# shubhamchandak94/HARC

Hardware: AMD Instinct MI355X
Metric: Mreads/s reorder+encode, 100 bp (higher is better)
Workload: dtype u64 (2-bit packed bases, XOR+popcount)

## Files before the change

### harc_amd/csrc/internal.h

```cpp
#pragma once
#include <hip/hip_runtime.h>
#include <stdint.h>
#include <stdio.h>
#include <string.h>
#include <map>
#include <string>
#include <utility>
#include <vector>
#include "../../include/harc_amd.h"

#define HARC_NONE 0xFFFFFFFFu
#define HARC_MAXW 8
#define HARC_MAXW3 12
#define HARC_MAXK (1u << 20)
#define HARC_LOOK_CHUNKS 16
#ifndef HARC_NSUGG
#define HARC_NSUGG 8
#endif

void harc_set_error(const char *fmt, ...);

#define HIP_TRY(expr)                                                                                          \
    do {                                                                                                       \
        hipError_t _e = (expr);                                                                                \
// ... 126 lines not shown
void harc_pool_release(harc_amd_ctx *c, harc_mark_t m);
struct PoolScope {
    harc_amd_ctx *c; harc_mark_t mk; bool armed = true;
    explicit PoolScope(harc_amd_ctx *c_) : c(c_), mk(harc_pool_mark(c_)) {}
    PoolScope(const PoolScope &) = delete;
    PoolScope &operator=(const PoolScope &) = delete;
    ~PoolScope() { if (armed) harc_pool_release(c, mk); }
    void keep() { armed = false; }
    void release_now() { if (armed) { harc_pool_release(c, mk); armed = false; } }
};

int prim_sort_pairs_u64_u32(harc_amd_ctx *c, const uint64_t *kin, uint64_t *kout, const uint32_t *vin, uint32_t *vout, size_t n, unsigned end_bit);
#define BL_TILE_WORDS 16384u
#define BL_PART_BITS 20
#define harc_bitmap_tiles(nwords) ((uint32_t)(((uint64_t)(nwords) + BL_TILE_WORDS - 1) / BL_TILE_WORDS))
#define harc_bitmap_item(w, b0, b1) (((uint64_t)((((uint32_t)(w) % BL_TILE_WORDS) << 10) | ((uint32_t)(b0) << 5) | (uint32_t)(b1)) << BL_PART_BITS) | (uint64_t)((uint32_t)(w) / BL_TILE_WORDS))
int harc_bitmap_from_items(harc_amd_ctx *c, const uint64_t *items, uint64_t *tmp, size_t n, uint64_t nwords, uint32_t *bitmap);
int prim_sort_keys_u64(harc_amd_ctx *c, const uint64_t *kin, uint64_t *kout, size_t n, unsigned end_bit);
int prim_excl_scan_u32(harc_amd_ctx *c, const uint32_t *in, uint32_t *out, size_t n);
int prim_excl_scan_u32_to_u64(harc_amd_ctx *c, const uint32_t *in, uint64_t *out, size_t n);
int prim_excl_scan_u8_to_u64(harc_amd_ctx *c, const uint8_t *in, uint64_t *out, size_t n);
int prim_incl_scan_u64(harc_amd_ctx *c, const uint64_t *in, uint64_t *out, size_t n);
int prim_incl_max_u32(harc_amd_ctx *c, const uint32_t *in, uint32_t *out, size_t n);
int prim_incl_max_u64(harc_amd_ctx *c, const uint64_t *in, uint64_t *out, size_t n);

int s1_pack_ascii(harc_amd_ctx *c, const char *d_ascii, uint32_t n, uint32_t stride, uint64_t *d_out);
int s1_pack3_ascii(harc_amd_ctx *c, const char *d_ascii, uint32_t n, uint32_t stride, uint64_t *d_out);
int s1_unpack_to_ascii(harc_amd_ctx *c, const uint64_t *d_reads, uint32_t n, char *d_out);
int s1_bucket_reads(harc_amd_ctx *c, const uint64_t *d_packed, uint32_t n, uint32_t nb, uint32_t *d_out);
int s1_partition_reads(harc_amd_ctx *c, const uint64_t *d_packed, uint32_t n, uint32_t nb, uint64_t *d_out, unsigned long long *d_counts);
int shard_partition(harc_amd_ctx *c, const uint64_t *d_words, uint32_t n, int nwords, bool three_bit, uint32_t nb, uint32_t gid0,
                    uint64_t *d_out, uint32_t *d_gid_out, unsigned long long *d_counts);
int shard_map_ids(harc_amd_ctx *c, uint32_t *d_v, uint64_t n, const uint32_t *d_map, uint32_t nmap, unsigned int *d_err);
int stage1_run(harc_amd_ctx *c);
int stage1_make_oriented(harc_amd_ctx *c, uint32_t i0 = 0, uint32_t i1 = 0xFFFFFFFFu);
int s1_orient(harc_amd_ctx *c, const uint64_t *reads, const uint32_t *order, const uint8_t *rc, uint32_t m, uint64_t *out);
int harc_dict_alloc(harc_amd_ctx *c, DictDev *d, uint32_t n, uint64_t cap_like);
int harc_dict_build(harc_amd_ctx *c, DictDev *d, uint64_t *keys, uint32_t *ids, uint32_t n, unsigned kbits);
void harc_dict_free(harc_amd_ctx *c, DictDev *d);
int stage2_run(harc_amd_ctx *c);
int pack_order_run(harc_amd_ctx *c);

static inline std::vector<uint8_t> &out_buf(harc_amd_ctx *c, int id, int shard) { harc_amd_ctx::OutBuf &o = c->out[std::make_pair(id, shard)]; o.ptr = nullptr; o.len = 0; return o.own; }
static inline void out_slice(harc_amd_ctx *c, int id, int shard, const void *p, size_t n) { harc_amd_ctx::OutBuf &o = c->out[std::make_pair(id, shard)]; o.own.clear(); o.ptr = (const uint8_t *)p; o.len = n; }
int harc_host_alloc(harc_amd_ctx *c, void **p, size_t bytes);
void harc_host_reset(harc_amd_ctx *c);
int harc_d2h(harc_amd_ctx *c, std::vector<uint8_t> &dst, const void *d_src, size_t bytes);

int build_line_index(harc_amd_ctx *c, const char *d_txt, uint64_t nbytes, const uint64_t **nls_out, uint64_t *total_lines_out);

int write_shard_family(harc_amd_ctx *c, const std::string &od, int first_shard, int e_lo = 0, int e_hi = -1);
int write_whole_job_files(harc_amd_ctx *c, const std::string &od);

struct BgzfCand { uint64_t off; uint32_t bsize, hdr, isize, crc; };
struct BgzfMember { uint64_t cdata, text; uint32_t clen, isize, crc, hdr; };
struct BgzfPlan { std::vector<BgzfMember> m; uint64_t text = 0, next = 0; };
int harc_bgzf_plan(harc_amd_ctx *c, const uint8_t *d_in, uint64_t n, uint64_t start, uint64_t own_end, uint64_t base_off, BgzfPlan *plan);
int harc_bgzf_run(harc_amd_ctx *c, const uint8_t *d_in, const BgzfPlan &plan, uint64_t base_off, char *d_out);

struct BgzfOutStats { uint64_t text = 0, bytes = 0, members = 0, stored = 0; double seconds = 0; };
int harc_bgzf_deflate(harc_amd_ctx *c, const char *d_text, uint64_t n_bytes, int32_t flags, uint8_t *d_out, uint64_t out_capacity, uint64_t *n_out, BgzfOutStats *st);
// ... 1 lines not shown
```

### harc_amd/csrc/prims.hip

```cpp
#include "devutil.h"
#include <rocprim/rocprim.hpp>

int harc_tmp_reserve(harc_amd_ctx *c, size_t bytes)
{
    if (bytes <= c->tmp_bytes) return HARC_AMD_OK;
    if (c->d_tmp) harc_raw_free(c, c->d_tmp);
    c->d_tmp = nullptr; c->tmp_bytes = 0;
    size_t want = bytes + (bytes >> 3) + 4096;
    RC_TRY(harc_raw_alloc(c, &c->d_tmp, want));
    c->tmp_bytes = want;
    return HARC_AMD_OK;
}

#define PRIM_CALL(call_with_tmp)                                \
    do {                                                        \
        size_t bytes = 0; void *tmp = nullptr;                  \
        HIP_TRY(call_with_tmp);                                 \
        RC_TRY(harc_tmp_reserve(c, bytes));                     \
        tmp = c->d_tmp; bytes = c->tmp_bytes;                   \
        HIP_TRY(call_with_tmp);                                 \
    } while (0)

int prim_sort_pairs_u64_u32(harc_amd_ctx *c, const uint64_t *kin, uint64_t *kout, const uint32_t *vin, uint32_t *vout, size_t n, unsigned end_bit)
{
// ... 32 lines not shown

int prim_excl_scan_u8_to_u64(harc_amd_ctx *c, const uint8_t *in, uint64_t *out, size_t n)
{
    if (n == 0) return HARC_AMD_OK;
    auto it = rocprim::make_transform_iterator(in, u8_to_u64());
    PRIM_CALL(rocprim::exclusive_scan(tmp, bytes, it, out, (uint64_t)0, n, rocprim::plus<uint64_t>(), c->stream));
    return HARC_AMD_OK;
}

int prim_incl_scan_u64(harc_amd_ctx *c, const uint64_t *in, uint64_t *out, size_t n)
{
    if (n == 0) return HARC_AMD_OK;
    PRIM_CALL(rocprim::inclusive_scan(tmp, bytes, in, out, n, rocprim::plus<uint64_t>(), c->stream));
    return HARC_AMD_OK;
}

int prim_incl_max_u32(harc_amd_ctx *c, const uint32_t *in, uint32_t *out, size_t n)
{
    if (n == 0) return HARC_AMD_OK;
    PRIM_CALL(rocprim::inclusive_scan(tmp, bytes, in, out, n, rocprim::maximum<uint32_t>(), c->stream));
    return HARC_AMD_OK;
}

int prim_incl_max_u64(harc_amd_ctx *c, const uint64_t *in, uint64_t *out, size_t n)
{
    if (n == 0) return HARC_AMD_OK;
    PRIM_CALL(rocprim::inclusive_scan(tmp, bytes, in, out, n, rocprim::maximum<uint64_t>(), c->stream));
    return HARC_AMD_OK;
}

__global__ void k_selftest_grid(uint64_t n, unsigned long long *out)
{
    const uint64_t i = harc_gid();
    unsigned long long one = i < n ? 1ULL : 0ULL, idx = i < n ? (unsigned long long)i : 0ULL;
    for (int o = 32; o > 0; o >>= 1) { one += __shfl_xor(one, o, 64); idx += __shfl_xor(idx, o, 64); }
    if ((threadIdx.x & 63) == 0 && one) { atomicAdd(&out[0], one); atomicAdd(&out[1], idx); }
}
__global__ void k_selftest_grid32(uint32_t n, unsigned long long *out)
{
    const uint32_t i = harc_gid32();
    unsigned long long one = i < n ? 1ULL : 0ULL, idx = i < n ? (unsigned long long)i : 0ULL;
    for (int o = 32; o > 0; o >>= 1) { one += __shfl_xor(one, o, 64); idx += __shfl_xor(idx, o, 64); }
    if ((threadIdx.x & 63) == 0 && one) { atomicAdd(&out[0], one); atomicAdd(&out[1], idx); }
}
__global__ void k_selftest_fold(uint64_t n, unsigned long long *out)
{
    const uint64_t wave = harc_bid() * 4 + (threadIdx.x >> 6);
    const int lane = threadIdx.x & 63;
    const uint64_t i = wave * 16 + (uint64_t)(lane >> 2);
    const bool mine = i < n && (lane & 3) == 0;
// ... 27 lines not shown
```

### harc_amd/csrc/stage1.hip

```cpp
#include "devutil.h"
#include <stdlib.h>
#include <type_traits>

struct S1Args {
    int L, maxmatch, thresh, maxsearch, Lp;
    int ds[2], de[2], kbits[2];
    uint32_t N, K;
    const uint64_t *reads;
    HashSlot *slots[2];
    uint64_t cap[2];
    const uint32_t *ids[2];
    int firstmax;
    const uint32_t *bloom[2]; uint32_t bloom_lines; int bloom_nwin[2]; uint32_t bloom_mmask;
    const uint2 *largetab;
    uint64_t *mirror;
    unsigned long long *claimed;
    uint32_t *bid;
    ChainHdr *hdr;
    uint4 *cnt;
    uint2 *steps;
    uint8_t *need;
    uint32_t *seedbuf;
    uint32_t *needrank;
    uint32_t *rmeta;
// ... 166 lines not shown
{
    const uint64_t gid = harc_gid();
    if (gid >= (uint64_t)n * W) return;
    const uint32_t i = (uint32_t)(gid / W); const int w = (int)(gid % W);
    out[gid] = reads[(size_t)idx[i] * W + w];
}
int s1_partition_reads(harc_amd_ctx *c, const uint64_t *d_packed, uint32_t n, uint32_t nb, uint64_t *d_out, unsigned long long *d_counts)
{
    HIP_TRY(hipMemsetAsync(d_counts, 0, (size_t)nb * 8, c->stream));
    if (!n) { HIP_TRY(hipStreamSynchronize(c->stream)); return HARC_AMD_OK; }
    PoolScope scope(c);
    uint32_t *b = nullptr, *i0 = nullptr, *i1 = nullptr; uint64_t *k0 = nullptr, *k1 = nullptr;
    RC_TRY(dalloc(c, &b, n)); RC_TRY(dalloc(c, &i0, n)); RC_TRY(dalloc(c, &i1, n)); RC_TRY(dalloc(c, &k0, n)); RC_TRY(dalloc(c, &k1, n));
    hipLaunchKernelGGL(k_bucket, harc_grid256(n), dim3(256), 0, c->stream, d_packed, n, c->P.readlen, c->W, nb, b);
    hipLaunchKernelGGL(k_bucket_keys, harc_grid256(n), dim3(256), 0, c->stream, (const uint32_t *)b, n, k0, i0, d_counts);
    unsigned bits = 1; while ((1u << bits) < nb) bits++;
    RC_TRY(prim_sort_pairs_u64_u32(c, k0, k1, i0, i1, n, bits));
    hipLaunchKernelGGL(k_gather_reads, harc_grid256((uint64_t)n * c->W), dim3(256), 0, c->stream, d_packed, (const uint32_t *)i1, n, c->W, d_out);
    HIP_TRY(hipGetLastError());
    HIP_TRY(hipStreamSynchronize(c->stream));
    return HARC_AMD_OK;
}

template <int W> __global__ void k_keygen2(const uint64_t *reads, uint32_t n, int off0, int nbits0, int off1, int nbits1, uint64_t *keys0, uint64_t *keys1, uint32_t *ids)
{
    const uint32_t i = harc_gid32();
    if (i >= n) return;
    uint64_t r[W];
#pragma unroll
    for (int w = 0; w < W; w++) r[w] = reads[(size_t)i * W + w];
    {
        const int wi = off0 >> 6, sh = off0 & 63;
        const uint64_t lo = sel0<W>(r, wi), hi = sel0<W>(r, wi + 1);
        uint64_t v = sh ? ((lo >> sh) | (hi << (64 - sh))) : lo;
        if (nbits0 < 64) v &= ((uint64_t)1 << nbits0) - 1;
        keys0[i] = v;
    }
    {
        const int wi = off1 >> 6, sh = off1 & 63;
        const uint64_t lo = sel0<W>(r, wi), hi = sel0<W>(r, wi + 1);
        uint64_t v = sh ? ((lo >> sh) | (hi << (64 - sh))) : lo;
        if (nbits1 < 64) v &= ((uint64_t)1 << nbits1) - 1;
        keys1[i] = v;
    }
    ids[i] = i;
}
__global__ void k_large_sizes(const unsigned long long *list, uint32_t nlist, HashSlot *s0, HashSlot *s1, uint32_t *sz)
{
    const uint32_t b = harc_gid32();
    if (b >= nlist) return;
    const unsigned long long e = list[b];
    const HashSlot *slot = ((e & 1) ? s1 : s0) + (e >> 1);
    sz[b] = slot->count & SLOT_CNT_MASK;
}
template <int W> __global__ __launch_bounds__(64) void k_large_fill(const unsigned long long *list, uint32_t nlist, HashSlot *s0, HashSlot *s1, const uint32_t *ids0, const uint32_t *ids1,
                                                                   const uint64_t *moff, const uint64_t *reads, uint2 *largetab, uint64_t *mirror)
{
    const uint32_t b = blockIdx.y * gridDim.x + blockIdx.x;
    if (b >= nlist) return;
    const int lane = threadIdx.x;
    const unsigned long long e = list[b];
    const int l = (int)(e & 1);
    HashSlot *slot = (l ? s1 : s0) + (e >> 1);
    const uint32_t st = slot->start, cnt = slot->count & SLOT_CNT_MASK;
    const uint32_t *ids = (l ? ids1 : ids0) + st;
    const uint64_t m0 = moff[b];
    for (uint32_t k = lane; k < cnt; k += 64) {
        const uint32_t rid = ids[k];
#pragma unroll
        for (int w = 0; w < W; w++) mirror[(m0 + k) * W + w] = reads[(size_t)rid * W + w];
    }
    if (lane == 0) { largetab[b] = make_uint2(st, (uint32_t)m0); slot->start = b; }
}
__global__ void k_mark_heads(const uint64_t *skeys, uint32_t n, uint32_t *head)
{
    const uint32_t i = harc_gid32();
    if (i >= n) return;
    head[i] = (i == 0 || skeys[i] != skeys[i - 1]) ? 1u : 0u;
}
__global__ void k_bin_starts(const uint32_t *head, const uint32_t *binidx, uint32_t n, uint32_t *binstart, uint32_t *nbins, const uint64_t *skeys, uint64_t cap, uint64_t *v)
{
    const uint32_t i = harc_gid32();
    if (i >= n) return;
    if (head[i]) { const uint32_t b = binidx[i]; binstart[b] = i; v[b] = bucket_slot(skeys[i], cap) + (uint64_t)n - (uint64_t)b; }
    if (i == n - 1) *nbins = binidx[i] + head[i];
}
#define HARC_LARGEBIN 16u
#define HARC_STEP_CAP 12
#define HARC_BO_FREE 1u
#define HARC_BO_CAP 3u
#define HARC_SCAN_BUDGET 12
#define MIXED_MAX (1u << 20)
#define MIXED_BUDGET 200000u
__device__ __forceinline__ uint64_t rotl64(uint64_t x, unsigned r) { r &= 63u; return r ? (x << r) | (x >> (64u - r)) : x; }
__global__ void k_mixed_find(const uint64_t *rk, uint32_t n, unsigned sbits, uint64_t *sk, uint32_t *list, unsigned int *meta)
{
    const uint32_t i = harc_gid32();
    if (i >= n) return;
    const int shift = (int)(64u - sbits);
    const uint64_t b = rotl64(rk[i], 64u - sbits);
    sk[i] = b;
    if (i == 0) return;
    const uint64_t a = rotl64(rk[i - 1], 64u - sbits);
    if (a != b && (a >> shift) == (b >> shift)) { const unsigned int at = atomicAdd(&meta[0], 1u); if (at < MIXED_MAX) list[at] = i; else meta[1] = 1u; }
}
__global__ void k_mixed_own(const uint64_t *sk, int shift, uint32_t *list, unsigned int *meta)
{
    const uint32_t t = harc_gid32();
    const unsigned int nl = meta[0] < MIXED_MAX ? meta[0] : MIXED_MAX;
    if (t >= nl || meta[1]) return;
    const uint32_t i = list[t];
    const uint64_t top = sk[i] >> shift;
    for (uint32_t h = i; h > 0 && (sk[h - 1] >> shift) == top;) {
        h--;
        if (h > 0 && sk[h] != sk[h - 1] && (sk[h - 1] >> shift) == top) { list[t] = HARC_NONE; return; }
        if (i - h > MIXED_BUDGET) { meta[1] = 1u; return; }
    }
// ... 85 lines not shown
                for (;;) {
                    unsigned long long *mp = reinterpret_cast<unsigned long long *>(&slots[sl]) + 1;
                    if (atomicCAS(mp, 0ULL, meta) == 0ULL) break;
                    if ((sl & 3) == 3) atomicOr(&slots[sl - 3].count, SLOT_OVF);
                    if (++sl == cap) sl = 0;
                }
                slots[sl].key = key;
            } else {
                uint4 w; w.x = (uint32_t)key; w.y = (uint32_t)(key >> 32); w.z = (uint32_t)meta; w.w = (uint32_t)(meta >> 32) | ovf;
                if (tiled) tile[sl - lo] = w; else *reinterpret_cast<uint4 *>(&slots[sl]) = w;
            }
            if (large_list && cnt > HARC_LARGEBIN) {
                const unsigned int at = atomicAdd(large_n, 1u);
                if (at < large_max) large_list[at] = ((unsigned long long)sl << 1) | large_tag;
            }
        }
    }
    if (tiled) {
        __syncthreads();
        for (uint32_t j = threadIdx.x; j < (uint32_t)(hi - lo); j += blockDim.x) *reinterpret_cast<uint4 *>(&slots[lo + j]) = tile[j];
    }
}

__global__ void k_s1_bloom_keys(const uint64_t *keys, uint32_t n, uint32_t nlines, int nwin, uint32_t mmask, uint64_t *pk)
{
    const uint32_t i = harc_gid32();
    if (i >= n) return;
    uint32_t w, m;
    bloom_pos(keys[i], key_scramble(keys[i]), nlines, nwin, mmask, &w, &m);
    const uint32_t b0 = (uint32_t)__ffs((int)m) - 1u, b1 = 31u - (uint32_t)__clz((int)m);
    pk[i] = harc_bitmap_item(w, b0, b1);
}
__global__ __launch_bounds__(256) void k_s1_bloom_tile(const uint64_t *pk, uint32_t n, uint64_t nwords, uint32_t *bloom)
{
    __shared__ uint32_t tile[BL_TILE_WORDS];
    __shared__ uint32_t bounds[2];
    const uint32_t part = blockIdx.x;
    for (uint32_t j = threadIdx.x; j < BL_TILE_WORDS; j += 256) tile[j] = 0u;
    if (threadIdx.x < 2) {
        const uint64_t want = (uint64_t)part + threadIdx.x, pmask = ((uint64_t)1 << BL_PART_BITS) - 1;
        uint32_t lo = 0, hi = n;
        while (lo < hi) { const uint32_t mid = lo + (hi - lo) / 2; if ((pk[mid] & pmask) < want) lo = mid + 1; else hi = mid; }
        bounds[threadIdx.x] = lo;
    }
    __syncthreads();
    for (uint32_t i = bounds[0] + threadIdx.x; i < bounds[1]; i += 256) {
        const uint32_t v = (uint32_t)(pk[i] >> BL_PART_BITS);
        atomicOr(&tile[v >> 10], (1u << ((v >> 5) & 31u)) | (1u << (v & 31u)));
    }
    __syncthreads();
    const uint64_t base = (uint64_t)part * BL_TILE_WORDS;
    for (uint32_t j = threadIdx.x; j < BL_TILE_WORDS; j += 256) if (base + j < nwords) bloom[base + j] = tile[j];
}
int harc_bitmap_from_items(harc_amd_ctx *c, const uint64_t *items, uint64_t *tmp, size_t n, uint64_t nwords, uint32_t *bitmap)
{
// ... 1936 lines not shown
    for (int k = 0; k < W; k++) r[k] = shfl_u64(mine, rl * W + k);
    if (!on) return;
    uint64_t ow = mine;
    if (rev) { rc_words<W>(r, L, o); ow = sel0<W>(o, w); }
    out[(size_t)i * W + w] = ow;
}

int harc_dict_alloc(harc_amd_ctx *c, DictDev *d, uint32_t n, uint64_t cap_like)
{
    d->cap = 0; d->slots = nullptr; d->ids = nullptr; d->d_nbins = nullptr;
    if (n == 0) return HARC_AMD_OK;
    if (cap_like) d->cap = cap_like;
    else {
        unsigned long long m = 4;
        size_t fr = 0, tot = 0;
        if (hipMemGetInfo(&fr, &tot) == hipSuccess) { fr += c->pool_total; while (m > 2 && ((double)m * n * sizeof(HashSlot) > 0.2 * (double)fr || (double)m * n * sizeof(HashSlot) > 0.15 * (double)tot)) m--; }
        if (c->P.table_slots_per_read >= 2 && c->P.table_slots_per_read <= 4) m = (unsigned long long)c->P.table_slots_per_read;
        if (const char *e = getenv("HARC_AMD_CAPMULT")) m = strtoull(e, nullptr, 10);
        d->cap = (((m < 2 ? 2 : m) * n + 4) + 3) & ~3ull;
    }
    RC_TRY(dalloc(c, &d->slots, d->cap)); RC_TRY(dalloc(c, &d->ids, n)); RC_TRY(dalloc(c, &d->d_nbins, 2));
    return HARC_AMD_OK;
}
int harc_dict_build(harc_amd_ctx *c, DictDev *d, uint64_t *keys, uint32_t *ids, uint32_t n, unsigned kbits)
{
    (void)kbits;
    if (n == 0) return HARC_AMD_OK;
    PoolScope scope(c);
    uint64_t *k1 = nullptr; uint32_t *h0 = nullptr, *b0 = nullptr, *bs = nullptr;
    RC_TRY(dalloc(c, &k1, n)); RC_TRY(dalloc(c, &h0, n)); RC_TRY(dalloc(c, &b0, n)); RC_TRY(dalloc(c, &bs, n));
    unsigned sbits = 64;
    { unsigned lg = 1; while (((uint64_t)1 << lg) < n) lg++; sbits = ((lg + 8 + 7) / 8) * 8; if (sbits > 64) sbits = 64; }
    if (const char *e = getenv("HARC_AMD_SORT_BITS")) { const int x = atoi(e); if (x >= 1 && x <= 64) sbits = (unsigned)x; }
    uint32_t *mixed = nullptr; unsigned int *mmeta = nullptr; uint64_t *k2 = nullptr;
    RC_TRY(dalloc(c, &mixed, MIXED_MAX)); RC_TRY(dalloc(c, &mmeta, 4));
    RC_TRY(dalloc(c, &k2, n));
    uint64_t *const k2v = k2;
    hipLaunchKernelGGL(k_scramble_keys, harc_grid256(n), dim3(256), 0, c->stream, keys, n, sbits < 64 ? sbits : 0u);
    uint32_t nbins = 0;
    for (;;) {
        HIP_TRY(hipMemsetAsync(mmeta, 0, 16, c->stream));
        HIP_TRY(hipMemsetAsync(d->d_nbins, 0, 8, c->stream));
        if (sbits < 64) {
            RC_TRY(prim_sort_pairs_u64_u32(c, keys, k2, ids, d->ids, n, sbits));
            hipLaunchKernelGGL(k_mixed_find, harc_grid256(n), dim3(256), 0, c->stream, (const uint64_t *)k2, n, sbits, k1, mixed, mmeta);
            hipLaunchKernelGGL(k_mixed_own, dim3(MIXED_MAX / 256), dim3(256), 0, c->stream, (const uint64_t *)k1, (int)(64 - sbits), mixed, mmeta);
            hipLaunchKernelGGL(k_mixed_fix, dim3(MIXED_MAX / 256), dim3(256), 0, c->stream, k1, d->ids, n, (int)(64 - sbits), (const uint32_t *)mixed, mmeta);
        } else RC_TRY(prim_sort_pairs_u64_u32(c, keys, k1, ids, d->ids, n, 64));
        hipLaunchKernelGGL(k_mark_heads, harc_grid256(n), dim3(256), 0, c->stream, k1, n, h0);
        RC_TRY(prim_excl_scan_u32(c, h0, b0, n));
        hipLaunchKernelGGL(k_bin_starts, harc_grid256(n), dim3(256), 0, c->stream, h0, b0, n, bs, d->d_nbins, (const uint64_t *)k1, d->cap, k2v);
        unsigned int mm[2] = { 0, 0 };
        HIP_TRY(hipMemcpyAsync(&nbins, d->d_nbins, 4, hipMemcpyDeviceToHost, c->stream));
        HIP_TRY(hipMemcpyAsync(mm, mmeta, 8, hipMemcpyDeviceToHost, c->stream));
        HIP_TRY(hipStreamSynchronize(c->stream));
        if (getenv("HARC_AMD_TRACE")) fprintf(stderr, "[index] sort on the top %u bits: %u places where different keys share them%s\n", sbits, mm[0], mm[1] ? " -- too many or too long, sorting on all bits" : "");
        if (!mm[1] || sbits == 64) break;
        hipLaunchKernelGGL(k_rotate_keys, harc_grid256(n), dim3(256), 0, c->stream, keys, n, 64u - sbits);
        sbits = 64;
    }
    const int fill = getenv("HARC_AMD_TABLE_FILL") ? atoi(getenv("HARC_AMD_TABLE_FILL")) != 0 : (uint64_t)nbins * 16 >= d->cap;
    if (!fill) HIP_TRY(hipMemsetAsync(d->slots, 0, d->cap * sizeof(HashSlot), c->stream));
    d->nbins = nbins;
    {
        uint64_t *v = k2v, *q = keys;
        const unsigned gb = (nbins + 255) / 256;
        RC_TRY(prim_incl_max_u64(c, v, q, nbins));
        for (int pass = 0; pass < 2; pass++)
            hipLaunchKernelGGL(k_table_place, dim3(gb), dim3(256), 0, c->stream, (const uint64_t *)k1, (const uint32_t *)d->ids, (const uint32_t *)bs, nbins, n, (const uint64_t *)q,
                               d->slots, d->cap, d->bigthresh, d->large_list, d->large_n, d->large_max, d->large_tag, d->d_nbins, pass, pass == 0 ? 0u : (gb > 64 ? gb - 64 : 0u), fill);
    }
    HIP_TRY(hipGetLastError());
    uint32_t nb2[2] = { 0, 0 };
    HIP_TRY(hipMemcpyAsync(nb2, d->d_nbins, 8, hipMemcpyDeviceToHost, c->stream));
    HIP_TRY(hipStreamSynchronize(c->stream));
    scope.release_now();
    if (nb2[1]) { harc_set_error("dictionary: %u bins hold more than %u reads with the same k-mer (count field of the slot), or lie more than 16384 bins beyond the end of the table", nb2[1], SLOT_CNT_MASK); return HARC_AMD_EINVAL; }
    return HARC_AMD_OK;
}
void harc_dict_free(harc_amd_ctx *c, DictDev *d)
{
    if (d->slots) harc_dev_free(c, d->slots);
    if (d->ids) harc_dev_free(c, d->ids);
    if (d->d_nbins) harc_dev_free(c, d->d_nbins);
    d->slots = nullptr; d->ids = nullptr; d->d_nbins = nullptr; d->cap = 0;
}

__global__ void k_selftest_ids(uint32_t *ids, uint32_t n)
{
    const uint32_t i = harc_gid32();
    if (i < n) ids[i] = i;
}
static int selftest_index(harc_amd_ctx *c, const uint64_t *keys, uint32_t n, uint32_t bigthresh, bool want_large, uint64_t *cap, uint32_t *nbins, void *slots,
                          uint32_t *ids, uint64_t *large, uint64_t large_capacity, uint64_t *n_large)
{
    PoolScope scope(c);
    DictDev d;
    RC_TRY(harc_dict_alloc(c, &d, n, 0));
    const uint64_t room = *cap;
    *cap = d.cap;
    if (!slots) return HARC_AMD_OK;
    if (room < d.cap) { harc_set_error("harc_amd_selftest_index: the table has %llu slots, the caller's buffer %llu", (unsigned long long)d.cap, (unsigned long long)room); return HARC_AMD_EINVAL; }
    uint64_t *k0 = nullptr; uint32_t *i0 = nullptr; unsigned long long *d_large = nullptr; unsigned int *d_nlarge = nullptr;
    const uint32_t maxlarge = 2 * (n / HARC_LARGEBIN) + 16;
    RC_TRY(dalloc(c, &k0, n)); RC_TRY(dalloc(c, &i0, n));
    if (want_large) {
        RC_TRY(dalloc(c, &d_large, maxlarge)); RC_TRY(dalloc(c, &d_nlarge, 4));
        HIP_TRY(hipMemsetAsync(d_nlarge, 0, 16, c->stream));
        d.large_list = d_large; d.large_n = d_nlarge; d.large_max = maxlarge; d.large_tag = 1u;
    }
    d.bigthresh = bigthresh;
    HIP_TRY(hipMemcpyAsync(k0, keys, (size_t)n * 8, hipMemcpyHostToDevice, c->stream));
    hipLaunchKernelGGL(k_selftest_ids, harc_grid256(n), dim3(256), 0, c->stream, i0, n);
    HIP_TRY(hipMemsetAsync(d.slots, 0xA5, d.cap * sizeof(HashSlot), c->stream));
    HIP_TRY(hipMemsetAsync(d.ids, 0xA5, (size_t)n * 4, c->stream));
    RC_TRY(harc_dict_build(c, &d, k0, i0, n, 64));
    *nbins = d.nbins;
    HIP_TRY(hipMemcpyAsync(slots, d.slots, d.cap * sizeof(HashSlot), hipMemcpyDeviceToHost, c->stream));
    HIP_TRY(hipMemcpyAsync(ids, d.ids, (size_t)n * 4, hipMemcpyDeviceToHost, c->stream));
    unsigned int nl = 0;
    if (want_large) HIP_TRY(hipMemcpyAsync(&nl, d_nlarge, 4, hipMemcpyDeviceToHost, c->stream));
    HIP_TRY(hipStreamSynchronize(c->stream));
    if (want_large) {
        *n_large = nl;
        uint64_t take = nl < maxlarge ? nl : maxlarge;
        if (take > large_capacity) take = large_capacity;
        if (take) HIP_TRY(hipMemcpy(large, d_large, (size_t)take * 8, hipMemcpyDeviceToHost));
    }
    return HARC_AMD_OK;
}
extern "C" int harc_amd_selftest_index(harc_amd_ctx *c, const uint64_t *keys, uint64_t n, int32_t slots_per_read, uint32_t bigthresh, int32_t want_large,
                                       uint64_t *cap, uint32_t *nbins, void *slots, uint32_t *ids, uint64_t *large, uint64_t large_capacity, uint64_t *n_large)
{
    if (!c || !cap || n == 0 || n > 0xFFFFFFF0ull || (slots_per_read != 0 && (slots_per_read < 2 || slots_per_read > 4))) { harc_set_error("harc_amd_selftest_index: bad arguments"); return HARC_AMD_EINVAL; }
    if (slots && (!keys || !nbins || !ids || (want_large && (!n_large || (!large && large_capacity))))) { harc_set_error("harc_amd_selftest_index: a NULL output"); return HARC_AMD_EINVAL; }
    HIP_TRY(hipSetDevice(c->P.device));
    const int32_t spr = c->P.table_slots_per_read;
    c->P.table_slots_per_read = slots_per_read;
    const int rc = selftest_index(c, keys, (uint32_t)n, bigthresh, want_large != 0, cap, nbins, slots, ids, large, large_capacity, n_large);
// ... 99 lines not shown
    unsigned long long *d_large = nullptr; unsigned int *d_nlarge = nullptr;
    const uint32_t maxlarge = 2 * (N / HARC_LARGEBIN) + 16;
    if (N) {
        RC_TRY(harc_dict_alloc(c, &dict[0], N, 0)); RC_TRY(harc_dict_alloc(c, &dict[1], N, dict[0].cap));
        ilap("tables allocated");
        RC_TRY(dalloc(c, &d_large, maxlarge)); RC_TRY(dalloc(c, &d_nlarge, 4));
        HIP_TRY(hipMemsetAsync(d_nlarge, 0, 16, c->stream));
        for (int l = 0; l < 2; l++) { dict[l].large_list = d_large; dict[l].large_n = d_nlarge; dict[l].large_max = maxlarge; dict[l].large_tag = (uint32_t)l; }
        dict[0].bigthresh = dict[1].bigthresh = HARC_LARGEBIN;
        if (bloom_bits) {
            uint64_t nl = ((uint64_t)N * (uint64_t)bloom_bits + 511) / 512 + 1;
            if (nl > 0x0FFFFFFFull) nl = 0x0FFFFFFFull;
            bloom_lines = (uint32_t)nl;
            bloom_tiled = getenv("HARC_AMD_S1BLOOM_TILED") ? atoi(getenv("HARC_AMD_S1BLOOM_TILED")) != 0 : (size_t)bloom_lines * 64 >= ((size_t)64 << 20);
            if (((uint64_t)bloom_lines * 16 + BL_TILE_WORDS - 1) / BL_TILE_WORDS + 1 >= ((uint64_t)1 << BL_PART_BITS)) bloom_tiled = false;
            for (int l = 0; l < 2; l++) {
                RC_TRY(dalloc(c, &d_bloom[l], (size_t)bloom_lines * 16)); if (!bloom_tiled) HIP_TRY(hipMemsetAsync(d_bloom[l], 0, (size_t)bloom_lines * 64, c->stream));
                const int nb = P.dict_end[l] - P.dict_start[l] + 1;
                const bool same = P.dict_end[0] - P.dict_start[0] == P.dict_end[1] - P.dict_start[1];
                bloom_nwin[l] = (same && bloom_m > 0 && nb > bloom_m && (size_t)bloom_lines * 64 >= bloom_mz_bytes) ? nb - bloom_m + 1 : 0;
            }
        }
        PoolScope kscope(c);
        uint64_t *kboth[2] = { nullptr, nullptr }; uint32_t *i0 = nullptr;
        RC_TRY(dalloc(c, &kboth[0], N)); RC_TRY(dalloc(c, &kboth[1], N)); RC_TRY(dalloc(c, &i0, N));
        hipLaunchKernelGGL((k_keygen2<W>), harc_grid256(N), dim3(256), 0, c->stream, c->d_reads, N, 2 * P.dict_start[0], 2 * (P.dict_end[0] - P.dict_start[0] + 1),
                           2 * P.dict_start[1], 2 * (P.dict_end[1] - P.dict_start[1] + 1), kboth[0], kboth[1], i0);
        ilap("bitmaps allocated, keys made");
        for (int l = 0; l < 2; l++) {
            const int kbits = 2 * (P.dict_end[l] - P.dict_start[l] + 1);
            uint64_t *const k0 = kboth[l];
            if (bloom_lines && bloom_tiled) {
                PoolScope bscope(c);
                uint64_t *pa = nullptr, *pb = nullptr; RC_TRY(dalloc(c, &pa, (size_t)N + 1)); RC_TRY(dalloc(c, &pb, (size_t)N + 1));
                const uint64_t nwords = (uint64_t)bloom_lines * 16;
                hipLaunchKernelGGL(k_s1_bloom_keys, harc_grid256(N), dim3(256), 0, c->stream, (const uint64_t *)k0, N, bloom_lines, bloom_nwin[l], bloom_mmask, pa);
                RC_TRY(harc_bitmap_from_items(c, pa, pb, N, nwords, d_bloom[l]));
                if (getenv("HARC_AMD_S1BLOOM_VERIFY")) {
                    uint32_t *ref = nullptr; unsigned long long *nd = nullptr, hnd = 0;
                    RC_TRY(dalloc(c, &ref, (size_t)nwords)); RC_TRY(dalloc(c, &nd, 1));
                    HIP_TRY(hipMemsetAsync(ref, 0, (size_t)nwords * 4, c->stream)); HIP_TRY(hipMemsetAsync(nd, 0, 8, c->stream));
                    hipLaunchKernelGGL(k_s1_bloom_set, harc_grid256(N), dim3(256), 0, c->stream, (const uint64_t *)k0, N, ref, bloom_lines, bloom_nwin[l], bloom_mmask);
                    hipLaunchKernelGGL(k_s1_bloom_diff, harc_grid256(nwords), dim3(256), 0, c->stream, (const uint32_t *)ref, (const uint32_t *)d_bloom[l], nwords, nd);
                    HIP_TRY(hipMemcpyAsync(&hnd, nd, 8, hipMemcpyDeviceToHost, c->stream));
                    HIP_TRY(hipStreamSynchronize(c->stream));
                    if (hnd) { harc_set_error("stage I bitmap built by tiles differs from the one built with atomics in %llu words", hnd); return HARC_AMD_EINTERNAL; }
                }
            } else if (bloom_lines) hipLaunchKernelGGL(k_s1_bloom_set, harc_grid256(N), dim3(256), 0, c->stream, (const uint64_t *)k0, N, d_bloom[l], bloom_lines, bloom_nwin[l], bloom_mmask);
            ilap("bitmap built");
            RC_TRY(harc_dict_build(c, &dict[l], k0, i0, N, (unsigned)kbits));
            ilap("table built");
        }
    }
    if (N && P.num_chains <= 0 && P.reads_per_chain <= 0 && (double)dict[0].nbins > 0.98 * (double)N) {
        const uint32_t k2 = N / 256 < 4096 ? N / 256 : 4096;
        if (k2 > K) { K = k2; c->C.chains = K; if (!getenv("HARC_AMD_QUAD")) quad = K <= 16384; }
    }
    uint32_t nlarge = 0;
    if (N) {
        HIP_TRY(hipMemcpyAsync(&nlarge, d_nlarge, 4, hipMemcpyDeviceToHost, c->stream));
        HIP_TRY(hipStreamSynchronize(c->stream));
        if (nlarge > maxlarge) { harc_set_error("stage I: %u bins above %u reads, list of %u", nlarge, HARC_LARGEBIN, maxlarge); return HARC_AMD_EINTERNAL; }
    }
    uint2 *d_largetab = nullptr; uint64_t *d_mirror = nullptr;
    uint32_t *d_sz0 = nullptr, *d_huge = nullptr; unsigned int *d_nhuge = nullptr; uint32_t nhuge = 0;
    uint64_t large_entries = 0;
    if (nlarge) {
        uint32_t *sz = nullptr; uint64_t *moff = nullptr;
        RC_TRY(dalloc(c, &d_largetab, nlarge)); RC_TRY(dalloc(c, &sz, (size_t)nlarge + 1)); RC_TRY(dalloc(c, &moff, (size_t)nlarge + 1));
        HIP_TRY(hipMemsetAsync(sz + nlarge, 0, 4, c->stream));
        hipLaunchKernelGGL(k_large_sizes, harc_grid256(nlarge), dim3(256), 0, c->stream, (const unsigned long long *)d_large, nlarge, dict[0].slots, dict[1].slots, sz);
        d_sz0 = sz;
        RC_TRY(dalloc(c, &d_huge, (size_t)nlarge + 1)); RC_TRY(dalloc(c, &d_nhuge, 4));
// ... 367 lines not shown
```

### harc_amd/csrc/stage2.hip

```cpp
#include "devutil.h"
#include <time.h>
#include <algorithm>
#include <stdlib.h>

#define TUPLE_NONE 0xFFFFFFFFFFFFFFFFULL

struct S2Args {
    int L, W, W3, thresh_s, maxsearch;
    int ds[2], de[2], kbits[2];
    uint32_t M, S, T, q, nC;
    uint64_t total;
    const uint64_t *oreads;
    const uint8_t *flag, *pos, *rc;
    const uint32_t *order;
    const uint64_t *cand3;
    const uint32_t *cand_order;
    uint8_t *head;
    uint64_t *gstart;
    uint8_t *cons;
    const uint32_t *chead;
    const HashSlot *slots[2]; uint64_t cap[2]; const uint32_t *ids[2];
    unsigned long long *best;
    unsigned long long *bestbin[2];
    const uint32_t *bloom[2]; int bloom_shift[2];
// ... 1477 lines not shown
            RC_TRY(dalloc(c, &bloom[0], ((size_t)1 << (lb - 3)) + 1));
            bloom4_tiled = getenv("HARC_AMD_S2BLOOM_TILED") ? atoi(getenv("HARC_AMD_S2BLOOM_TILED")) != 0 : (((size_t)1 << (lb - 3)) * 4 >= ((size_t)64 << 20));
            if ((uint64_t)T * 4 > 0xFFFFFFFFull || harc_bitmap_tiles((uint64_t)1 << (lb - 3)) + 1 >= (1u << BL_PART_BITS)) bloom4_tiled = false;
            if (!bloom4_tiled) HIP_TRY(hipMemsetAsync(bloom[0], 0, ((size_t)1 << (lb - 3)) * 4, c->stream));
            bloom[1] = bloom[0]; bloom_shift[0] = bloom_shift[1] = 64 - lb;
            a.bloom_lbits = lb - 7;
            a.bloom_nwin = (a.kbits[0] / 3 == 21 && !getenv("HARC_AMD_BLOOM4_HASHED")) ? 21 - BLOOM4_M + 1 : 0;
        } else for (int l = 0; l < 2; l++) {
            RC_TRY(dalloc(c, &bloom[l], ((size_t)1 << (lb - 5)) + 1));
            HIP_TRY(hipMemsetAsync(bloom[l], 0, ((size_t)1 << (lb - 5)) * 4, c->stream));
            bloom_shift[l] = 64 - lb;
        }
        PoolScope kscope(c);
        uint64_t *k0 = nullptr; uint32_t *i0k = nullptr; uint64_t *items = nullptr, *items_tmp = nullptr;
        RC_TRY(dalloc(c, &k0, T)); RC_TRY(dalloc(c, &i0k, T));
        const uint64_t b4words = (uint64_t)1 << (lb - 3);
        if (bloom4 && bloom4_tiled) { RC_TRY(dalloc(c, &items, (size_t)T * 4 + 1)); RC_TRY(dalloc(c, &items_tmp, (size_t)T * 4 + 1)); }
        for (int l = 0; l < 2; l++) {
            hipLaunchKernelGGL(k_key3, G256(T), cand3, T, W3, 3 * a.ds[l], a.kbits[l], k0, i0k);
            if (bloom4 && bloom4_tiled) hipLaunchKernelGGL(k_bloom4_items, G256(T), (const uint64_t *)k0, T, a.bloom_lbits, a.bloom_nwin, l, a.kbits[l] / 3, harc_bitmap_tiles(b4words), items + (size_t)l * 2 * T);
            else if (bloom4) hipLaunchKernelGGL(k_bloom4_set, G256(T), (const uint64_t *)k0, T, bloom[0], a.bloom_lbits, a.bloom_nwin, l, a.kbits[l] / 3);
            else hipLaunchKernelGGL(k_bloom_set, G256(T), (const uint64_t *)k0, T, bloom[l], bloom_shift[l]);
            lap("  keys, bitmap items");
            RC_TRY(harc_dict_build(c, &dict[l], k0, i0k, T, (unsigned)a.kbits[l]));
            hipLaunchKernelGGL(k_count_big_bins, G256(dict[l].cap), dict[l].slots, dict[l].cap, (uint32_t)P.maxsearch, d_big);
            lap("  dictionary built");
        }
        if (bloom4 && bloom4_tiled) {
            RC_TRY(harc_bitmap_from_items(c, items, items_tmp, (size_t)T * 4, b4words, bloom[0]));
            lap("  combined bitmap from sorted items");
            if (getenv("HARC_AMD_S2BLOOM_VERIFY")) {
                uint32_t *ref = nullptr; unsigned long long *nd = nullptr, hnd = 0;
                RC_TRY(dalloc(c, &ref, (size_t)b4words + 1)); RC_TRY(dalloc(c, &nd, 1));
                HIP_TRY(hipMemsetAsync(ref, 0, (size_t)b4words * 4, c->stream)); HIP_TRY(hipMemsetAsync(nd, 0, 8, c->stream));
                for (int l = 0; l < 2; l++) {
                    hipLaunchKernelGGL(k_key3, G256(T), cand3, T, W3, 3 * a.ds[l], a.kbits[l], k0, i0k);
                    hipLaunchKernelGGL(k_bloom4_set, G256(T), (const uint64_t *)k0, T, ref, a.bloom_lbits, a.bloom_nwin, l, a.kbits[l] / 3);
                }
                hipLaunchKernelGGL(k_words_differ, harc_grid256(b4words), dim3(256), 0, c->stream, (const uint32_t *)ref, (const uint32_t *)bloom[0], b4words, nd);
                HIP_TRY(hipMemcpyAsync(&hnd, nd, 8, hipMemcpyDeviceToHost, c->stream));
                HIP_TRY(hipStreamSynchronize(c->stream));
                if (hnd) { harc_set_error("stage II bitmap built by tiles differs from the one built with atomics in %llu words", hnd); return HARC_AMD_EINTERNAL; }
            }
        }
        HIP_TRY(hipStreamSynchronize(c->stream));
    }
    for (int l = 0; l < 2; l++) { a.slots[l] = dict[l].slots; a.cap[l] = dict[l].cap; a.ids[l] = dict[l].ids; a.bloom[l] = bloom[l]; a.bloom_shift[l] = bloom_shift[l]; }
// ... 437 lines not shown
```

Before: 695.7.

## Fuse key scrambling and bloom items into keygen, single-pass bin scan in dict build

Stage I key generation now produces the scrambled, rotated sortable keys and the bloom bitmap items (or atomic bloom bits) in the same kernel, so the separate scramble and bloom-key kernels and their extra passes over the key arrays go away. Dictionary building swaps the head-mark, exclusive-scan, bin-start and inclusive-max chain for a custom two-pass wavefront scan that finds bin heads, ranks and the running max of slot offsets together. This cuts kernel launches and global memory traffic, but the bin scan adds a decoupled segment scan that leans on the MIXED scratch buffer and wave-level shuffles, which brings correctness and capacity risks.

```diff
diff --git a/harc_amd/csrc/internal.h b/harc_amd/csrc/internal.h
--- a/harc_amd/csrc/internal.h
+++ b/harc_amd/csrc/internal.h
@@ -172,7 +172,7 @@
 int prim_excl_scan_u8_to_u64(harc_amd_ctx *c, const uint8_t *in, uint64_t *out, size_t n);
 int prim_incl_scan_u64(harc_amd_ctx *c, const uint64_t *in, uint64_t *out, size_t n);
 int prim_incl_max_u32(harc_amd_ctx *c, const uint32_t *in, uint32_t *out, size_t n);
-int prim_incl_max_u64(harc_amd_ctx *c, const uint64_t *in, uint64_t *out, size_t n);
+int prim_bins_scan(harc_amd_ctx *c, const uint64_t *skeys, size_t n, uint64_t cap, uint32_t *binstart, uint64_t *q, uint32_t *nbins, void *scratch, size_t scratch_bytes);
 
 int s1_pack_ascii(harc_amd_ctx *c, const char *d_ascii, uint32_t n, uint32_t stride, uint64_t *d_out);
 int s1_pack3_ascii(harc_amd_ctx *c, const char *d_ascii, uint32_t n, uint32_t stride, uint64_t *d_out);
@@ -186,7 +186,9 @@
 int stage1_make_oriented(harc_amd_ctx *c, uint32_t i0 = 0, uint32_t i1 = 0xFFFFFFFFu);
 int s1_orient(harc_amd_ctx *c, const uint64_t *reads, const uint32_t *order, const uint8_t *rc, uint32_t m, uint64_t *out);
 int harc_dict_alloc(harc_amd_ctx *c, DictDev *d, uint32_t n, uint64_t cap_like);
-int harc_dict_build(harc_amd_ctx *c, DictDev *d, uint64_t *keys, uint32_t *ids, uint32_t n, unsigned kbits);
+enum { HARC_KEYS_RAW = 0, HARC_KEYS_SORTABLE = 1 };
+unsigned harc_dict_sort_bits(uint32_t n);
+int harc_dict_build(harc_amd_ctx *c, DictDev *d, uint64_t *keys, uint32_t *ids, uint32_t n, unsigned kbits, int keys_are);
 void harc_dict_free(harc_amd_ctx *c, DictDev *d);
 int stage2_run(harc_amd_ctx *c);
 int pack_order_run(harc_amd_ctx *c);
diff --git a/harc_amd/csrc/prims.hip b/harc_amd/csrc/prims.hip
--- a/harc_amd/csrc/prims.hip
+++ b/harc_amd/csrc/prims.hip
@@ -78,10 +78,72 @@
     return HARC_AMD_OK;
 }
 
-int prim_incl_max_u64(harc_amd_ctx *c, const uint64_t *in, uint64_t *out, size_t n)
+struct BinPart { long long m; uint32_t c, pad; };
+struct BinPartOp {
+    __host__ __device__ BinPart operator()(const BinPart &a, const BinPart &b) const
+    {
+        const long long bm = b.m - (long long)a.c;
+        return BinPart{ a.m > bm ? a.m : bm, a.c + b.c, 0u };
+    }
+};
+#define BINS_NONE (-(1ll << 62))
+#define BINS_SEG_MIN 2048u
+#define BINS_UNROLL 4
+template <bool WRITE> __global__ __launch_bounds__(256) void k_bins_pass(const uint64_t *k, uint32_t n, uint64_t cap, uint32_t seg, uint32_t nseg, BinPart *part,
+                                                                       uint32_t *binstart, uint64_t *q, uint32_t *nbins)
+{
+    const uint32_t w = (blockIdx.x * 256u + threadIdx.x) >> 6;
+    if (w >= nseg) return;
+    const int lane = threadIdx.x & 63;
+    const unsigned long long below = ((unsigned long long)1 << lane) - 1;
+    uint32_t C = 0; long long M = BINS_NONE;
+    if (WRITE) { C = part[w].c; M = part[w].m; }
+    const uint64_t base = (uint64_t)w * seg, end = base + seg < n ? base + seg : (uint64_t)n;
+    uint64_t carry = base ? k[base - 1] : 0;
+    for (uint64_t at = base; at < end; at += 64u * BINS_UNROLL) {
+        uint64_t key[BINS_UNROLL];
+#pragma unroll
+        for (int u = 0; u < BINS_UNROLL; u++) { const uint64_t i = at + 64u * u + lane; key[u] = i < end ? k[i] : 0; }
+#pragma unroll
+        for (int u = 0; u < BINS_UNROLL; u++) {
+            const uint64_t i = at + 64u * u + lane;
+            uint64_t prev = __shfl_up(key[u], 1, 64);
+            if (lane == 0) prev = carry;
+            carry = __shfl(key[u], 63, 64);
+            const bool head = i < end && (i == 0 || key[u] != prev);
+            const unsigned long long hb = __ballot(head);
+            const uint32_t rank = C + (uint32_t)__popcll(hb & below);
+            long long v = head ? (long long)bucket_slot(key[u], cap) - (long long)rank : BINS_NONE;
+            if (WRITE) {
+                for (int d = 1; d < 64; d <<= 1) { const long long o = __shfl_up(v, d, 64); if (lane >= d && o > v) v = o; }
+                if (M > v) v = M;
+                if (head) { binstart[rank] = (uint32_t)i; q[rank] = (uint64_t)(v + (long long)n); }
+                if (i < end && i + 1 == n) *nbins = rank + (head ? 1u : 0u);
+                M = __shfl(v, 63, 64);
+            } else if (v > M) M = v;
+            C += (uint32_t)__popcll(hb);
+        }
+    }
+    if (!WRITE) {
+        for (int o = 32; o > 0; o >>= 1) { const long long x = __shfl_xor(M, o, 64); if (x > M) M = x; }
+        if (lane == 0) part[w] = BinPart{ M, C, 0u };
+    }
+}
+int prim_bins_scan(harc_amd_ctx *c, const uint64_t *skeys, size_t n, uint64_t cap, uint32_t *binstart, uint64_t *q, uint32_t *nbins, void *scratch, size_t scratch_bytes)
 {
     if (n == 0) return HARC_AMD_OK;
-    PRIM_CALL(rocprim::inclusive_scan(tmp, bytes, in, out, n, rocprim::maximum<uint64_t>(), c->stream));
+    const size_t room = scratch_bytes / (2 * sizeof(BinPart));
+    if (room == 0 || n > 0xFFFFFFFFull || (n + room - 1) / room > (1u << 30) || room > 0x7FFFFFFFull) { harc_set_error("prim_bins_scan: %zu keys, scratch of %zu bytes", n, scratch_bytes); return HARC_AMD_EINVAL; }
+    size_t seg = (n + room - 1) / room;
+    if (seg < BINS_SEG_MIN) seg = BINS_SEG_MIN;
+    seg = (seg + 64 * BINS_UNROLL - 1) / (64 * BINS_UNROLL) * (64 * BINS_UNROLL);
+    const uint32_t nseg = (uint32_t)((n + seg - 1) / seg);
+    BinPart *part = (BinPart *)scratch, *front = part + nseg;
+    const dim3 grid((nseg + 3) / 4);
+    hipLaunchKernelGGL(k_bins_pass<false>, grid, dim3(256), 0, c->stream, skeys, (uint32_t)n, cap, (uint32_t)seg, nseg, part, (uint32_t *)nullptr, (uint64_t *)nullptr, (uint32_t *)nullptr);
+    PRIM_CALL(rocprim::exclusive_scan(tmp, bytes, part, front, BinPart{ BINS_NONE, 0u, 0u }, (size_t)nseg, BinPartOp(), c->stream));
+    hipLaunchKernelGGL(k_bins_pass<true>, grid, dim3(256), 0, c->stream, skeys, (uint32_t)n, cap, (uint32_t)seg, nseg, front, binstart, q, nbins);
+    HIP_TRY(hipGetLastError());
     return HARC_AMD_OK;
 }
 
diff --git a/harc_amd/csrc/stage1.hip b/harc_amd/csrc/stage1.hip
--- a/harc_amd/csrc/stage1.hip
+++ b/harc_amd/csrc/stage1.hip
@@ -212,27 +212,35 @@
     return HARC_AMD_OK;
 }
 
-template <int W> __global__ void k_keygen2(const uint64_t *reads, uint32_t n, int off0, int nbits0, int off1, int nbits1, uint64_t *keys0, uint64_t *keys1, uint32_t *ids)
+__device__ __forceinline__ uint64_t rotl64(uint64_t x, unsigned r) { r &= 63u; return r ? (x << r) | (x >> (64u - r)) : x; }
+struct KeyOut { uint64_t *keys, *items; uint32_t *bloom; int off, nbits, nwin; };
+template <int W, bool RAW> __device__ __forceinline__ void keygen_one(const uint64_t (&r)[W], uint32_t i, const KeyOut &o, unsigned rot, uint32_t nlines, uint32_t mmask)
+{
+    const int wi = o.off >> 6, sh = o.off & 63;
+    const uint64_t lo = sel0<W>(r, wi), hi = sel0<W>(r, wi + 1);
+    uint64_t v = sh ? ((lo >> sh) | (hi << (64 - sh))) : lo;
+    if (o.nbits < 64) v &= ((uint64_t)1 << o.nbits) - 1;
+    if constexpr (RAW) o.keys[i] = v;
+    else {
+        const uint64_t hk = key_scramble(v);
+        o.keys[i] = rotl64(hk, rot);
+        if (o.items || o.bloom) {
+            uint32_t w, m;
+            bloom_pos(v, hk, nlines, o.nwin, mmask, &w, &m);
+            if (o.items) { const uint32_t b0 = (uint32_t)__ffs((int)m) - 1u, b1 = 31u - (uint32_t)__clz((int)m); o.items[i] = harc_bitmap_item(w, b0, b1); }
+            else if ((o.bloom[w] & m) != m) atomicOr(&o.bloom[w], m);
+        }
+    }
+}
+template <int W, bool RAW> __global__ void k_keygen2(const uint64_t *reads, uint32_t n, KeyOut o0, KeyOut o1, uint32_t *ids, unsigned rot, uint32_t nlines, uint32_t mmask)
 {
     const uint32_t i = harc_gid32();
     if (i >= n) return;
     uint64_t r[W];
 #pragma unroll
     for (int w = 0; w < W; w++) r[w] = reads[(size_t)i * W + w];
-    {
-        const int wi = off0 >> 6, sh = off0 & 63;
-        const uint64_t lo = sel0<W>(r, wi), hi = sel0<W>(r, wi + 1);
-        uint64_t v = sh ? ((lo >> sh) | (hi << (64 - sh))) : lo;
-        if (nbits0 < 64) v &= ((uint64_t)1 << nbits0) - 1;
-        keys0[i] = v;
-    }
-    {
-        const int wi = off1 >> 6, sh = off1 & 63;
-        const uint64_t lo = sel0<W>(r, wi), hi = sel0<W>(r, wi + 1);
-        uint64_t v = sh ? ((lo >> sh) | (hi << (64 - sh))) : lo;
-        if (nbits1 < 64) v &= ((uint64_t)1 << nbits1) - 1;
-        keys1[i] = v;
-    }
+    keygen_one<W, RAW>(r, i, o0, rot, nlines, mmask);
+    keygen_one<W, RAW>(r, i, o1, rot, nlines, mmask);
     ids[i] = i;
 }
 __global__ void k_large_sizes(const unsigned long long *list, uint32_t nlist, HashSlot *s0, HashSlot *s1, uint32_t *sz)
@@ -262,19 +270,6 @@
     }
     if (lane == 0) { largetab[b] = make_uint2(st, (uint32_t)m0); slot->start = b; }
 }
-__global__ void k_mark_heads(const uint64_t *skeys, uint32_t n, uint32_t *head)
-{
-    const uint32_t i = harc_gid32();
-    if (i >= n) return;
-    head[i] = (i == 0 || skeys[i] != skeys[i - 1]) ? 1u : 0u;
-}
-__global__ void k_bin_starts(const uint32_t *head, const uint32_t *binidx, uint32_t n, uint32_t *binstart, uint32_t *nbins, const uint64_t *skeys, uint64_t cap, uint64_t *v)
-{
-    const uint32_t i = harc_gid32();
-    if (i >= n) return;
-    if (head[i]) { const uint32_t b = binidx[i]; binstart[b] = i; v[b] = bucket_slot(skeys[i], cap) + (uint64_t)n - (uint64_t)b; }
-    if (i == n - 1) *nbins = binidx[i] + head[i];
-}
 #define HARC_LARGEBIN 16u
 #define HARC_STEP_CAP 12
 #define HARC_BO_FREE 1u
@@ -282,7 +277,6 @@
 #define HARC_SCAN_BUDGET 12
 #define MIXED_MAX (1u << 20)
 #define MIXED_BUDGET 200000u
-__device__ __forceinline__ uint64_t rotl64(uint64_t x, unsigned r) { r &= 63u; return r ? (x << r) | (x >> (64u - r)) : x; }
 __global__ void k_mixed_find(const uint64_t *rk, uint32_t n, unsigned sbits, uint64_t *sk, uint32_t *list, unsigned int *meta)
 {
     const uint32_t i = harc_gid32();
@@ -414,15 +408,6 @@
     }
 }
 
-__global__ void k_s1_bloom_keys(const uint64_t *keys, uint32_t n, uint32_t nlines, int nwin, uint32_t mmask, uint64_t *pk)
-{
-    const uint32_t i = harc_gid32();
-    if (i >= n) return;
-    uint32_t w, m;
-    bloom_pos(keys[i], key_scramble(keys[i]), nlines, nwin, mmask, &w, &m);
-    const uint32_t b0 = (uint32_t)__ffs((int)m) - 1u, b1 = 31u - (uint32_t)__clz((int)m);
-    pk[i] = harc_bitmap_item(w, b0, b1);
-}
 __global__ __launch_bounds__(256) void k_s1_bloom_tile(const uint64_t *pk, uint32_t n, uint64_t nwords, uint32_t *bloom)
 {
     __shared__ uint32_t tile[BL_TILE_WORDS];
@@ -2405,21 +2390,25 @@
     RC_TRY(dalloc(c, &d->slots, d->cap)); RC_TRY(dalloc(c, &d->ids, n)); RC_TRY(dalloc(c, &d->d_nbins, 2));
     return HARC_AMD_OK;
 }
-int harc_dict_build(harc_amd_ctx *c, DictDev *d, uint64_t *keys, uint32_t *ids, uint32_t n, unsigned kbits)
+unsigned harc_dict_sort_bits(uint32_t n)
+{
+    unsigned lg = 1; while (((uint64_t)1 << lg) < n) lg++;
+    unsigned sbits = ((lg + 8 + 7) / 8) * 8; if (sbits > 64) sbits = 64;
+    if (const char *e = getenv("HARC_AMD_SORT_BITS")) { const int x = atoi(e); if (x >= 1 && x <= 64) sbits = (unsigned)x; }
+    return sbits;
+}
+int harc_dict_build(harc_amd_ctx *c, DictDev *d, uint64_t *keys, uint32_t *ids, uint32_t n, unsigned kbits, int keys_are)
 {
     (void)kbits;
     if (n == 0) return HARC_AMD_OK;
     PoolScope scope(c);
-    uint64_t *k1 = nullptr; uint32_t *h0 = nullptr, *b0 = nullptr, *bs = nullptr;
-    RC_TRY(dalloc(c, &k1, n)); RC_TRY(dalloc(c, &h0, n)); RC_TRY(dalloc(c, &b0, n)); RC_TRY(dalloc(c, &bs, n));
-    unsigned sbits = 64;
-    { unsigned lg = 1; while (((uint64_t)1 << lg) < n) lg++; sbits = ((lg + 8 + 7) / 8) * 8; if (sbits > 64) sbits = 64; }
-    if (const char *e = getenv("HARC_AMD_SORT_BITS")) { const int x = atoi(e); if (x >= 1 && x <= 64) sbits = (unsigned)x; }
+    uint64_t *k1 = nullptr; uint32_t *bs = nullptr;
+    RC_TRY(dalloc(c, &k1, n)); RC_TRY(dalloc(c, &bs, n));
+    unsigned sbits = harc_dict_sort_bits(n);
     uint32_t *mixed = nullptr; unsigned int *mmeta = nullptr; uint64_t *k2 = nullptr;
     RC_TRY(dalloc(c, &mixed, MIXED_MAX)); RC_TRY(dalloc(c, &mmeta, 4));
     RC_TRY(dalloc(c, &k2, n));
-    uint64_t *const k2v = k2;
-    hipLaunchKernelGGL(k_scramble_keys, harc_grid256(n), dim3(256), 0, c->stream, keys, n, sbits < 64 ? sbits : 0u);
+    if (keys_are == HARC_KEYS_RAW) hipLaunchKernelGGL(k_scramble_keys, harc_grid256(n), dim3(256), 0, c->stream, keys, n, sbits);
     uint32_t nbins = 0;
     for (;;) {
         HIP_TRY(hipMemsetAsync(mmeta, 0, 16, c->stream));
@@ -2430,9 +2419,7 @@
             hipLaunchKernelGGL(k_mixed_own, dim3(MIXED_MAX / 256), dim3(256), 0, c->stream, (const uint64_t *)k1, (int)(64 - sbits), mixed, mmeta);
             hipLaunchKernelGGL(k_mixed_fix, dim3(MIXED_MAX / 256), dim3(256), 0, c->stream, k1, d->ids, n, (int)(64 - sbits), (const uint32_t *)mixed, mmeta);
         } else RC_TRY(prim_sort_pairs_u64_u32(c, keys, k1, ids, d->ids, n, 64));
-        hipLaunchKernelGGL(k_mark_heads, harc_grid256(n), dim3(256), 0, c->stream, k1, n, h0);
-        RC_TRY(prim_excl_scan_u32(c, h0, b0, n));
-        hipLaunchKernelGGL(k_bin_starts, harc_grid256(n), dim3(256), 0, c->stream, h0, b0, n, bs, d->d_nbins, (const uint64_t *)k1, d->cap, k2v);
+        RC_TRY(prim_bins_scan(c, k1, n, d->cap, bs, k2, d->d_nbins, mixed, (size_t)MIXED_MAX * sizeof(uint32_t)));
         unsigned int mm[2] = { 0, 0 };
         HIP_TRY(hipMemcpyAsync(&nbins, d->d_nbins, 4, hipMemcpyDeviceToHost, c->stream));
         HIP_TRY(hipMemcpyAsync(mm, mmeta, 8, hipMemcpyDeviceToHost, c->stream));
@@ -2446,11 +2433,10 @@
     if (!fill) HIP_TRY(hipMemsetAsync(d->slots, 0, d->cap * sizeof(HashSlot), c->stream));
     d->nbins = nbins;
     {
-        uint64_t *v = k2v, *q = keys;
+        const uint64_t *q = k2;
         const unsigned gb = (nbins + 255) / 256;
-        RC_TRY(prim_incl_max_u64(c, v, q, nbins));
         for (int pass = 0; pass < 2; pass++)
-            hipLaunchKernelGGL(k_table_place, dim3(gb), dim3(256), 0, c->stream, (const uint64_t *)k1, (const uint32_t *)d->ids, (const uint32_t *)bs, nbins, n, (const uint64_t *)q,
+            hipLaunchKernelGGL(k_table_place, dim3(gb), dim3(256), 0, c->stream, (const uint64_t *)k1, (const uint32_t *)d->ids, (const uint32_t *)bs, nbins, n, q,
                                d->slots, d->cap, d->bigthresh, d->large_list, d->large_n, d->large_max, d->large_tag, d->d_nbins, pass, pass == 0 ? 0u : (gb > 64 ? gb - 64 : 0u), fill);
     }
     HIP_TRY(hipGetLastError());
@@ -2497,7 +2483,7 @@
     hipLaunchKernelGGL(k_selftest_ids, harc_grid256(n), dim3(256), 0, c->stream, i0, n);
     HIP_TRY(hipMemsetAsync(d.slots, 0xA5, d.cap * sizeof(HashSlot), c->stream));
     HIP_TRY(hipMemsetAsync(d.ids, 0xA5, (size_t)n * 4, c->stream));
-    RC_TRY(harc_dict_build(c, &d, k0, i0, n, 64));
+    RC_TRY(harc_dict_build(c, &d, k0, i0, n, 64, HARC_KEYS_RAW));
     *nbins = d.nbins;
     HIP_TRY(hipMemcpyAsync(slots, d.slots, d.cap * sizeof(HashSlot), hipMemcpyDeviceToHost, c->stream));
     HIP_TRY(hipMemcpyAsync(ids, d.ids, (size_t)n * 4, hipMemcpyDeviceToHost, c->stream));
@@ -2643,33 +2629,41 @@
             }
         }
         PoolScope kscope(c);
-        uint64_t *kboth[2] = { nullptr, nullptr }; uint32_t *i0 = nullptr;
+        uint64_t *kboth[2] = { nullptr, nullptr }, *items[2] = { nullptr, nullptr }; uint32_t *i0 = nullptr;
         RC_TRY(dalloc(c, &kboth[0], N)); RC_TRY(dalloc(c, &kboth[1], N)); RC_TRY(dalloc(c, &i0, N));
-        hipLaunchKernelGGL((k_keygen2<W>), harc_grid256(N), dim3(256), 0, c->stream, c->d_reads, N, 2 * P.dict_start[0], 2 * (P.dict_end[0] - P.dict_start[0] + 1),
-                           2 * P.dict_start[1], 2 * (P.dict_end[1] - P.dict_start[1] + 1), kboth[0], kboth[1], i0);
+        const bool by_items = bloom_lines && bloom_tiled;
+        if (by_items) RC_TRY(dalloc(c, &items[1], N));
+        const harc_mark_t mark_items1 = harc_pool_mark(c);
+        if (by_items) RC_TRY(dalloc(c, &items[0], N));
+        KeyOut ko[2];
+        for (int l = 0; l < 2; l++)
+            ko[l] = KeyOut{ kboth[l], items[l], (bloom_lines && !by_items) ? d_bloom[l] : nullptr, 2 * P.dict_start[l], 2 * (P.dict_end[l] - P.dict_start[l] + 1), bloom_nwin[l] };
+        hipLaunchKernelGGL((k_keygen2<W, false>), harc_grid256(N), dim3(256), 0, c->stream, c->d_reads, N, ko[0], ko[1], i0, harc_dict_sort_bits(N), bloom_lines, bloom_mmask);
         ilap("bitmaps allocated, keys made");
         for (int l = 0; l < 2; l++) {
             const int kbits = 2 * (P.dict_end[l] - P.dict_start[l] + 1);
-            uint64_t *const k0 = kboth[l];
-            if (bloom_lines && bloom_tiled) {
+            if (by_items) {
                 PoolScope bscope(c);
-                uint64_t *pa = nullptr, *pb = nullptr; RC_TRY(dalloc(c, &pa, (size_t)N + 1)); RC_TRY(dalloc(c, &pb, (size_t)N + 1));
+                uint64_t *pb = nullptr; RC_TRY(dalloc(c, &pb, (size_t)N + 1));
                 const uint64_t nwords = (uint64_t)bloom_lines * 16;
-                hipLaunchKernelGGL(k_s1_bloom_keys, harc_grid256(N), dim3(256), 0, c->stream, (const uint64_t *)k0, N, bloom_lines, bloom_nwin[l], bloom_mmask, pa);
-                RC_TRY(harc_bitmap_from_items(c, pa, pb, N, nwords, d_bloom[l]));
+                RC_TRY(harc_bitmap_from_items(c, items[l], pb, N, nwords, d_bloom[l]));
                 if (getenv("HARC_AMD_S1BLOOM_VERIFY")) {
-                    uint32_t *ref = nullptr; unsigned long long *nd = nullptr, hnd = 0;
-                    RC_TRY(dalloc(c, &ref, (size_t)nwords)); RC_TRY(dalloc(c, &nd, 1));
+                    uint32_t *ref = nullptr, *ri = nullptr; unsigned long long *nd = nullptr, hnd = 0; uint64_t *raw[2] = { nullptr, nullptr };
+                    RC_TRY(dalloc(c, &ref, (size_t)nwords)); RC_TRY(dalloc(c, &nd, 1)); RC_TRY(dalloc(c, &raw[0], N)); RC_TRY(dalloc(c, &raw[1], N)); RC_TRY(dalloc(c, &ri, N));
                     HIP_TRY(hipMemsetAsync(ref, 0, (size_t)nwords * 4, c->stream)); HIP_TRY(hipMemsetAsync(nd, 0, 8, c->stream));
-                    hipLaunchKernelGGL(k_s1_bloom_set, harc_grid256(N), dim3(256), 0, c->stream, (const uint64_t *)k0, N, ref, bloom_lines, bloom_nwin[l], bloom_mmask);
+                    KeyOut kr[2] = { ko[0], ko[1] };
+                    for (int x = 0; x < 2; x++) { kr[x].keys = raw[x]; kr[x].items = nullptr; kr[x].bloom = nullptr; }
+                    hipLaunchKernelGGL((k_keygen2<W, true>), harc_grid256(N), dim3(256), 0, c->stream, c->d_reads, N, kr[0], kr[1], ri, 0u, 0u, 0u);
+                    hipLaunchKernelGGL(k_s1_bloom_set, harc_grid256(N), dim3(256), 0, c->stream, (const uint64_t *)raw[l], N, ref, bloom_lines, bloom_nwin[l], bloom_mmask);
                     hipLaunchKernelGGL(k_s1_bloom_diff, harc_grid256(nwords), dim3(256), 0, c->stream, (const uint32_t *)ref, (const uint32_t *)d_bloom[l], nwords, nd);
                     HIP_TRY(hipMemcpyAsync(&hnd, nd, 8, hipMemcpyDeviceToHost, c->stream));
                     HIP_TRY(hipStreamSynchronize(c->stream));
                     if (hnd) { harc_set_error("stage I bitmap built by tiles differs from the one built with atomics in %llu words", hnd); return HARC_AMD_EINTERNAL; }
                 }
-            } else if (bloom_lines) hipLaunchKernelGGL(k_s1_bloom_set, harc_grid256(N), dim3(256), 0, c->stream, (const uint64_t *)k0, N, d_bloom[l], bloom_lines, bloom_nwin[l], bloom_mmask);
+            }
+            if (l == 0) harc_pool_release(c, mark_items1);
             ilap("bitmap built");
-            RC_TRY(harc_dict_build(c, &dict[l], k0, i0, N, (unsigned)kbits));
+            RC_TRY(harc_dict_build(c, &dict[l], kboth[l], i0, N, (unsigned)kbits, HARC_KEYS_SORTABLE));
             ilap("table built");
         }
     }
diff --git a/harc_amd/csrc/stage2.hip b/harc_amd/csrc/stage2.hip
--- a/harc_amd/csrc/stage2.hip
+++ b/harc_amd/csrc/stage2.hip
@@ -1523,7 +1523,7 @@
             else if (bloom4) hipLaunchKernelGGL(k_bloom4_set, G256(T), (const uint64_t *)k0, T, bloom[0], a.bloom_lbits, a.bloom_nwin, l, a.kbits[l] / 3);
             else hipLaunchKernelGGL(k_bloom_set, G256(T), (const uint64_t *)k0, T, bloom[l], bloom_shift[l]);
             lap("  keys, bitmap items");
-            RC_TRY(harc_dict_build(c, &dict[l], k0, i0k, T, (unsigned)a.kbits[l]));
+            RC_TRY(harc_dict_build(c, &dict[l], k0, i0k, T, (unsigned)a.kbits[l], HARC_KEYS_RAW));
             hipLaunchKernelGGL(k_count_big_bins, G256(dict[l].cap), dict[l].slots, dict[l].cap, (uint32_t)P.maxsearch, d_big);
             lap("  dictionary built");
         }
```

Result: faster. 710.5, median of 6 (+2.1%).
